# hidasib/GRU4Rec

Measured on AMD Instinct MI355X. Metric: mini-batches/sec (gru4rec.py:661), RSC15-shaped batch=128 n_sample=2048 BPR-max, higher is better.
Workload: dtype f32

## Files before the change

### gru4rec_amd/build.py

```python
import glob
import os
import subprocess
import sys

HERE = os.path.dirname(os.path.abspath(__file__))
SRC = os.path.join(HERE, 'csrc', 'g4r_api.hip')
SRC_HOST = os.path.join(HERE, 'csrc', 'g4r_io.cpp')
OUT = os.path.join(HERE, 'libgru4rec_hip.so')
DEPS = sorted(p for ext in ('hip', 'cuh', 'hpp', 'cpp') for p in glob.glob(os.path.join(HERE, 'csrc', '*.' + ext))) + \
       [os.path.join(os.path.dirname(HERE), 'include', 'gru4rec_hip.h'), os.path.abspath(__file__)]


def build(force=False, verbose=False, out=None, defs=(), flags=()):
    if out is not None:
        return _compile(out, list(defs), verbose, list(flags))
    if not force and os.path.exists(OUT) and all(os.path.getmtime(OUT) >= os.path.getmtime(d) for d in DEPS):
        return OUT
    return _compile(OUT, [], verbose)


COMMON_FLAGS = ['-mllvm', '-amdgpu-kernarg-preload-count=16']


MUTANTS = {1: 'sparse accumulator increments x 1.01', 2: 'sparse Adagrad steps x 1.01', 3: 'dense accumulator increments x 1.01',
# ... 7 lines not shown
           10: "k_replay_final (g4r_recommend_sessions) reads every row's final state from the buffer of the chunk's LONGEST history",
           11: "k_score_cand (g4r_score_candidates*): a work item past a row's first slice reads the items of the row's first slice",
           12: "the two-stage top-k (g4r_recommend_*_scan) ranks its candidates by the APPROXIMATE bf16 scores: the fp32 re-scoring is skipped",
           13: "cosine (g4r_similar_items): the candidate's inverse norm is read at the candidate POSITION instead of its item index",
           14: "k_rollout_feed (g4r_continue_sessions): the sorted insertion drops an item that sorts ABOVE every item already in the row's "
               "exclusion list, so it is never excluded and can be generated again",
           15: "k_beam_advance (g4r_beam_sessions) reads the hidden state of beam row i ITSELF instead of the row of its parent: a new beam "
               "carries on from the wrong state wherever the selection re-parents",
           16: "the owner walk of k_sparse_update_generic drops the first hit of every pass after the first (an item with more than 64 "
               "earlier occurrences in a step loses one of them per later pass)",
           17: "opt_rule's new second statistic (adadelta's update average, Adam's mean) x 1.01",
           18: "k_loss_rows' grp_fast takes a group of V columns whose last column is the first inactive in-batch one (column M) as wholly "
               "active: the unmasked copy of the element loops runs over it",
           19: "k_loss_rows' first pass starts its loop past the prefetched groups one STEP late: the columns of the first trip keep "
               "whatever the LDS held",
           20: "gumbel_noise (g4r_sample_sessions) ignores the decoding step (Philox counter word 2 = 0): every step of a draw gets the "
               "noise of step 0",
           21: "k_owner_window takes the sample-store row of every step of its window from the window's FIRST global step: the owner "
               "tables of the later steps are those of another list",
           22: "hidden_act_bwd decides the branch of leaky / elu / selu on the VALUE of the stored candidate (c >= 0), not on its sign bit: "
               "a pre-activation whose result rounds to -0.0 gets the positive branch's slope",
           23: "hidden_act_bwd: the negative-branch slope of leaky / elu / selu x 1.01",
           24: "k_mmr_rerank (g4r_diversify_*): from the second update on, a position's largest similarity to the picks is OVERWRITTEN by "
               "its similarity to the last pick instead of max-ed with it"}


def mutant_path(k):
    return os.path.join(HERE, '_variants', 'libgru4rec_hip_mut%d.so' % k)


def build_mutants(force=False, verbose=False):
    import fcntl
    from concurrent.futures import ThreadPoolExecutor
    os.makedirs(os.path.join(HERE, '_variants'), exist_ok=True)

    def stale():
        return [k for k in MUTANTS if force or not os.path.exists(mutant_path(k)) or
                any(os.path.getmtime(mutant_path(k)) < os.path.getmtime(d) for d in DEPS)]
    if not stale():
        return [mutant_path(k) for k in MUTANTS]
    with open(os.path.join(HERE, '_variants', '.lock'), 'w') as lock:
        fcntl.flock(lock, fcntl.LOCK_EX)
        todo = stale()
        if todo:
            _host_object(verbose)
            with ThreadPoolExecutor(min(len(todo), 2)) as ex:
                list(ex.map(lambda k: _device(mutant_path(k), ['G4R_MUTATE=%d' % k], verbose, audit=(k != 4)), todo))
# ... 108 lines not shown
```

### gru4rec_amd/csrc/g4r_host_create.hpp

```cpp

int g4r_device_count(void) {
    int n = 0;
    if (hipGetDeviceCount(&n) != hipSuccess) return 0;
    return n;
}
const char* g4r_last_error(void) { return g_err.c_str(); }
#ifndef G4R_HIPCC_VERSION
#define G4R_HIPCC_VERSION "unknown"
#endif
const char* g4r_version(void) { return "gru4rec_hip 0.4 (gfx950; hipcc " G4R_HIPCC_VERSION "; isa-audited)"; }
int g4r_sizeof_config(void) { return (int)sizeof(g4r_config); }

static int build_lean_args(g4r_model* m) {
    DevModel& d = m->dm;
    const StepKernels& k = m->kern;
    const int L = d.n_layers;
    std::vector<LeanV> av(L); std::vector<LeanH> ah(L); std::vector<LeanDa> aa(L); std::vector<LeanDy> ay(L);
    const bool constrained = d.embed_mode == G4R_EMBED_CONSTRAINED;
    bool any_layer = false;
    for (int l = 0; l < L; ++l) {
        if (k.fwd[l] != FWD_LEAN) continue;
        any_layer = true;
        LeanV& v = av[l]; memset(&v, 0, sizeof(v));
        v.Wx = d.dense_p + d.offWx[l]; v.Wrz = d.dense_p + d.offWrz[l]; v.Bh = d.dense_p + d.offBh[l];
// ... 52 lines not shown
        u.lr = d.lr; u.mom = d.mom; u.lmbd = d.lmbd;
        m->h_leanU = u;
        const std::vector<DenseTile> tiles = dense_tiles(d, 16, 64);
        m->ntiles16 = (int)tiles.size();
        const size_t nslot = cdiv((long long)G4R_OWN_SLOTS * d.R * 16 * sizeof(int), (long long)sizeof(DenseTile));
        if (dalloc(m, &m->d_tiles16, tiles.size() + nslot) || dalloc(m, &m->d_leanU, (size_t)1)) return -1;
        d.own_pos = m->sw.owner_scan_in_update ? nullptr : (int*)(m->d_tiles16 + tiles.size());
        m->h_leanU.own_on = d.own_pos ? 1 : 0;
        const bool pays = cdiv(d.R, LOSS_NW) > G4R_OWN_WINDOW_MINWG;
        m->own_window = d.own_pos && d.R <= G4R_OWN_WINDOW_MAXR && (m->sw.owner_window > 0 || (m->sw.owner_window < 0 && pays));
        HIPCHK(hipMemcpyAsync(m->d_tiles16, tiles.data(), tiles.size() * sizeof(DenseTile), hipMemcpyHostToDevice, m->stream));
        HIPCHK(hipStreamSynchronize(m->stream));
    }
    HIPCHK(hipStreamSynchronize(m->stream));
    return 0;
}

static KernelSwitches read_switches(const g4r_config& cfg) {
    KernelSwitches w;
    w.no_lean = getenv("G4R_NO_LEAN") != nullptr; w.no_mt = getenv("G4R_NO_MT") != nullptr; w.no_bmt = getenv("G4R_NO_BMT") != nullptr;
    w.no_merge = getenv("G4R_NO_MERGE") != nullptr; w.owner_scan_in_update = env_int("G4R_OWNER_SCAN", 0) != 0;
    w.owner_window = env_int("G4R_OWNER_WINDOW", -1);
    w.score_b_split = env_int("G4R_SCORE_B_SPLIT", 1) != 0;
    w.allow_lean_update = env_int("G4R_LEAN_UPDATE", 1) != 0; w.defer = env_int("G4R_DEFER", cfg.defer_updates) != 0;
    w.p2_geo = env_int("G4R_P2_GEO", -1); w.ba_geo = env_int("G4R_BA_GEO", -1);
    w.wide2 = env_int("G4R_WIDE2", -1); w.p1_ks = env_int("G4R_P1_KS", 128); w.bb_ks = env_int("G4R_BB_KS", 0);
    const char* skip = getenv("G4R_SKIP_KN");
    w.skip_kn = skip ? strtoull(skip, nullptr, 0) : 0ull;
    w.trace = getenv("G4R_TRACE") != nullptr;
    return w;
}

int g4r_create(const g4r_config* cfg, g4r_model** out) {
    if (!cfg || !out) return fail("null argument");
    if (cfg->n_layers < 1 || cfg->n_layers > G4R_MAX_LAYERS) return fail("n_layers out of range");
    if (cfg->batch_size < 1 || cfg->n_items < 1) return fail("batch_size / n_items must be positive");
    for (int l = 0; l < cfg->n_layers; ++l)
        if (cfg->layers[l] % 4 != 0 || cfg->layers[l] < 4 || cfg->layers[l] > 1024)
            return fail("layer sizes must be multiples of 4 in [4, 1024]");
    if (cfg->embed_mode == G4R_EMBED_SEPARATE && (cfg->embedding % 4 != 0 || cfg->embedding < 4 || cfg->embedding > 1024))
        return fail("embedding must be a multiple of 4 in [4, 1024]");
    if (cfg->embed_mode != G4R_EMBED_CONSTRAINED && cfg->embed_mode != G4R_EMBED_SEPARATE && cfg->embed_mode != G4R_EMBED_ONEHOT)
        return fail("unsupported embedding mode");
    if (cfg->embed_mode == G4R_EMBED_ONEHOT && 3 * cfg->layers[0] > 1024)
        return fail("one-hot input: 3 * layers[0] must be <= 1024 (row width of the Wx[0] table)");
    if (cfg->loss < 0 || cfg->loss > G4R_LOSS_XE_LOGIT) return fail("unsupported loss");
// ... 224 lines not shown
```

### gru4rec_amd/csrc/g4r_host_debug.hpp

```cpp
int g4r_get_debug(g4r_model* m, const char* name, float* host, int64_t count) {
    if (!m || !name || !host) return fail("null argument");
    HIPCHK(hipSetDevice(m->cfg.device));
    DevModel& d = m->dm;
    const StepKernels& k = m->kern;
    std::string s(name);
    const float* p = nullptr; int64_t n = 0;
    int l = 0;
    if (!s.empty() && isdigit((unsigned char)s.back())) { l = s.back() - '0'; s.pop_back(); }
    if (l >= d.n_layers) return fail("layer out of range");
    const int64_t bd = (int64_t)d.B * d.D[l];
    if (s == "scores") { p = d.Sc; n = (int64_t)d.B * d.ldSc; }
    else if (s == "dSx") { p = d.dSx + (size_t)((m->gstep - 1) & d.defer_mask) * (size_t)d.dSx_stride; n = (int64_t)d.B * d.Ein; }
    else if (s == "dSy") { p = d.dSy + (size_t)((m->gstep - 1) & d.defer_mask) * (size_t)d.dSy_stride; n = (int64_t)d.ldSc * d.Dtop; }
    else if (s == "dSBy") { p = d.dSBy + (size_t)((m->gstep - 1) & d.defer_mask) * (size_t)d.dSBy_stride; n = d.ldSc; }
    else if (s == "defer_stats") {
        if (count < 4) return fail("count");
        double rows = 0, bias = 0;
        if (m->defer_on) {
            std::vector<unsigned> st(2048);
            HIPCHK(hipStreamSynchronize(m->stream));
            HIPCHK(hipMemcpy(st.data(), d.dstat, st.size() * sizeof(unsigned), hipMemcpyDeviceToHost));
            for (size_t i = 0; i < st.size(); i += 2) { rows += st[i]; bias += st[i + 1]; }
        }
        host[0] = (float)rows; host[1] = (float)bias; host[2] = m->defer_on ? 1.f : 0.f; host[3] = (float)(d.defer_mask + 1);
// ... 55 lines not shown
        host[0] = (float)(k.p2_deep[0] + 2 * k.ba_deep[0]); return 0;
    }
    else if (s == "score_mt") { if (count < 1) return fail("count"); host[0] = k.score_fwd == SF_MT ? 272.f : 0.f; return 0; }
    else if (s == "score_bmt") { if (count < 1) return fail("count"); host[0] = (float)k.bmt_slabs; return 0; }
    else if (s == "lean") {
        if (count < 4) return fail("count");
        int mk = 0;
        for (int l = 0; l < d.n_layers; ++l) mk |= k.fwd[l] == FWD_LEAN ? 1 << l : 0;
        host[0] = (float)mk; host[1] = k.score_fwd == SF_LEAN ? 1.f : 0.f; host[2] = k.score_bwd == SB_LEAN ? 1.f : 0.f;
        host[3] = k.update == UP_LEAN ? 1.f : 0.f;
        return 0;
    }
    else if (s == "kernels") {
        const int ML = G4R_MAX_LAYERS;
        const int tail[] = {k.score_fwd, k.loss_spec, k.loss_long, k.loss_quads, k.score_bwd, k.kch, k.ksplit, k.bmt_slabs, k.update, k.chunks, k.wide_dense, k.finish_rows};
        if (count < 4 * ML + 12) return fail("count");
        for (int i = 0; i < 4 * ML + 12; ++i) host[i] = i < 4 * ML ? 0.f : (float)tail[i - 4 * ML];
        for (int l = 0; l < d.n_layers; ++l) {
            host[l] = (float)k.fwd[l]; host[ML + l] = (float)k.bwd[l]; host[2 * ML + l] = (float)(k.p2_deep[l] + 2 * k.ba_deep[l]); host[3 * ML + l] = (float)k.wg[l].use;
        }
        return 0;
    }
    else if (s == "generic") { if (count < 1) return fail("count"); host[0] = (float)d.generic; return 0; }
    else if (s == "score_b_split") { if (count < 1) return fail("count"); host[0] = (float)k.score_a_host; return 0; }
    else if (s == "n_cu") { if (count < 1) return fail("count"); host[0] = (float)m->n_cu; return 0; }
    else if (s == "ksplit") { if (count < 1) return fail("count"); host[0] = (float)d.ksplit; return 0; }
    else if (s == "dev_syncs") { if (count < 1) return fail("count"); host[0] = (float)m->n_dev_syncs; return 0; }
    else if (s == "dense_count") { if (count < 1) return fail("count"); host[0] = (float)d.dense_count; return 0; }
    else if (s == "occ_score_tile") {
        if (count < 1) return fail("count");
        int nb = 0;
        for (size_t lds = SMEM_SF2; lds >= SMEM_SF2 - 2048; lds -= 512) {
            HIPCHK(hipOccupancyMaxActiveBlocksPerMultiprocessor(&nb, (const void*)k_score_fwd_t2, GT_NTH, lds));
            fprintf(stderr, "[g4r] k_score_fwd_t2 dynamic LDS %zu -> %d workgroups per CU\n", lds, nb);
        }
        host[0] = (float)nb;
        return 0;
    }
    else if (s == "graph_mode") {
        if (count < 1) return fail("count");
        host[0] = m->gexec ? 1.f : (m->gexec_head ? 2.f : 0.f);
        return 0;
    }
    else return fail(std::string("unknown debug buffer ") + name);
    if (count != n) return fail(std::string("size mismatch for debug buffer ") + name + " expected " + std::to_string(n));
    HIPCHK(hipStreamSynchronize(m->stream));
// ... 169 lines not shown
```

### gru4rec_amd/csrc/g4r_host_model.hpp

```cpp
static thread_local std::string g_err;
static int fail(const std::string& s) { g_err = s; return -1; }
void g4r_set_error(const char* fmt, ...) {
    char buf[1024];
    va_list ap;
    va_start(ap, fmt);
    vsnprintf(buf, sizeof(buf), fmt, ap);
    va_end(ap);
    g_err = buf;
}
#define HIPCHK(x)                                                                                        \
    do {                                                                                                 \
        hipError_t e_ = (x);                                                                             \
        if (e_ != hipSuccess)                                                                            \
            return fail(std::string(#x) + ": " + hipGetErrorString(e_) + " @" + std::to_string(__LINE__)); \
    } while (0)
#define NCCLCHK(x)                                                                                         \
    do {                                                                                                   \
        ncclResult_t e_ = (x);                                                                             \
        if (e_ != ncclSuccess)                                                                             \
            return fail(std::string(#x) + ": " + ncclGetErrorString(e_) + " @" + std::to_string(__LINE__)); \
    } while (0)

enum { KN_GRU_P1 = 0, KN_GRU_P2, KN_SCORE_FWD, KN_LOSS, KN_SCORE_BWD, KN_BWD_PRE, KN_BWD_A, KN_BWD_B, KN_DENSE, KN_ALLREDUCE,
       KN_DENSE_APPLY, KN_SPARSE, KN_UPDATE, KN_BWD_FUSED, KN_FWD_FUSED, KN_GATE, KN_FLUSH, KN_SCAN, KN_FINISH, KN_GRU_V, KN_GRU_H, KN_GRU_DA, KN_GRU_DY, KN_OWNER_WINDOW, KN_COUNT };
static const char* KN_NAMES[KN_COUNT] = {"k_gru_p1", "k_gru_p2", "k_score_fwd", "k_loss_rows", "k_score_bwd", "k_gru_bwd_pre",
                                         "k_gru_bwd_a", "k_gru_bwd_b", "k_dense_grad", "rccl_allreduce", "k_dense_apply",
                                         "k_sparse_update", "k_update", "k_gru_bwd", "k_gru_fwd", "k_gru_gate", "k_sparse_flush", "k_defer_scan", "k_finish_rows", "k_gru_v", "k_gru_h", "k_gru_da", "k_gru_dy", "k_owner_window"};

struct EvRec { int kn; hipEvent_t a, b; };

struct KernelSwitches {
    bool no_lean = false;
    bool no_mt = false, no_bmt = false;
    bool no_merge = false;
    bool allow_lean_update = true;
    bool score_b_split = true;
    bool owner_scan_in_update = false;
    int owner_window = -1;
    bool defer = false;
    int p2_geo = -1, ba_geo = -1;
    int wide2 = -1, p1_ks = 128, bb_ks = 0;
    unsigned long long skip_kn = 0;
    bool trace = false;
};
enum GruFwdKind { FWD_LEAN = 0 , FWD_FUSED = 1 , FWD_P1S = 2 ,
                  FWD_P1_N64 = 3, FWD_P1_N32 = 4 };
enum GruBwdKind { BWD_LEAN = 0 , BWD_FUSED = 1 , BWD_ONEHOT = 2, BWD_BW = 3, BWD_B = 4 };
enum ScoreFwdKind { SF_LEAN = 0 , SF_MT = 1 , SF_T3 = 2, SF_T2 = 3, SF_K64 = 4, SF_K128 = 5  };
enum ScoreBwdKind { SB_LEAN = 0 , SB_BMT = 1 , SB_BWD2 = 2 , SB_W = 3, SB_N = 4  };
enum UpdateKind { UP_LEAN = 0 , UP_MERGED = 1 , UP_SPLIT = 2 };
struct WideGeo { int use = 0, ny = 1, nh = 1, kys = 0, khs = 0, bbn = 1, bbk = 0; };
struct StepKernels {
    int fwd[G4R_MAX_LAYERS], bwd[G4R_MAX_LAYERS];
    int p2_deep[G4R_MAX_LAYERS], ba_deep[G4R_MAX_LAYERS];
    WideGeo wg[G4R_MAX_LAYERS];
    int score_fwd;
    int loss_spec, loss_long, loss_quads;
    int score_bwd;
    int score_a_host;
    int kch, ksplit;
    int bmt_slabs;
    int nblkA, nblkB, ndtA, ndtB, nrtB;
    int update;
    int chunks;
    int wide_dense;
    int finish_rows;
};

template <class T>
struct DevBuf {
    T* p = nullptr;
    int64_t cap = 0;
    int reserve(g4r_model* m, int64_t n);
};

struct g4r_model {
    g4r_config cfg;
    DevModel dm;
    DevModel* d_dm = nullptr;
    int n_cu = 256;
    KernelSwitches sw;
    StepKernels kern;
// ... 323 lines not shown
    const bool wide = (B >= 256 && d.ldSc >= 4096) || (Dt % 64 == 0 && B >= 192 && d.ldSc >= 2048);
    const bool dma = Dt % 32 == 0 && (wide || (Dt >= 256 && B >= 64 && d.ldSc >= 1024));
    bool mt = false;
    if (!sw.no_mt && dma && Dt % 32 == 0 && Dt >= 32 && n_cu / cdiv(B, 64) >= 1) {
        const int nrb = cdiv(B, 64), W = 16 * cdiv(d.ldSc, 16 * (n_cu / nrb));
        mt = W == 272 && nrb * cdiv(d.ldSc, W) * 8 >= n_cu * 7;
    }
    const bool lean_s = !sw.no_lean && Dt <= LN_MAXD && Dt % 4 == 0 && !wide && !dma && B < 65536 && d.ldSc < 65536;
    k.score_fwd = lean_s ? SF_LEAN : mt ? SF_MT : dma ? SF_T3 : (wide && Dt % T2_BK == 0) ? SF_T2 : wide ? SF_K64 : SF_K128;
    k.loss_spec = (d.final_act == G4R_ACT_ELU && d.loss == G4R_LOSS_BPR_MAX) ? 1 : (d.final_act == G4R_ACT_SOFTMAX && d.loss == G4R_LOSS_XE) ? 2
                : (d.final_act == G4R_ACT_ELU && d.loss == G4R_LOSS_TOP1_MAX) ? 3 : 0;
    k.loss_long = (size_t)(2 * d.ldSc + 18 * LOSS_NW) * sizeof(float) > (size_t)(156 * 1024);
    k.loss_quads = d.ldSc >= 4 * LOSS_T;
    const bool bwd2 = wide && Dt % 64 == 0;
    const bool top_tiles = k.bwd[top] != BWD_LEAN && k.bwd[top] != BWD_FUSED;
    if (!sw.no_bmt && bwd2 && top_tiles && Dt % 128 == 0 && Dt <= 512 && d.ldSc % BMT_WA == 0 && d.ldSc <= 0xFFFF && B <= 0xFFFF) {
        const int ntA = d.ldSc / BMT_WA * (Dt / 32), den = cdiv(B, 64) * (Dt / 128), ks = ntA / den;
        if (ntA % den == 0 && ntA % 8 == 0 && ntA <= n_cu && ntA * 8 >= n_cu * 7 && BMT_WA % (Dt / 32) == 0 && 4 * (BMT_WA / (Dt / 32)) <= 256 &&
            ks >= 2 && ks <= 24 && d.ldSc % ks == 0 && (d.ldSc / ks) % 32 == 0 && d.ldSc / ks <= 2048)
            k.bmt_slabs = ks;
    }
    k.score_bwd = (lean_s && B <= 128) ? SB_LEAN : k.bmt_slabs ? SB_BMT : bwd2 ? SB_BWD2 : wide ? SB_W : SB_N;
    k.score_a_host = (sw.score_b_split && k.score_bwd == SB_LEAN && k.bwd[top] == BWD_LEAN) ? 1 : 0;
    const int slabs_target = top_tiles ? 17 : 9;
    k.kch = GT_BK * std::max(1, (cdiv(d.ldSc, GT_BK) + slabs_target / 2) / slabs_target);
    if (k.score_bwd == SB_LEAN) k.kch = 128;
    else if (k.score_bwd == SB_BMT) k.kch = d.ldSc / k.bmt_slabs;
    else if (k.score_bwd == SB_BWD2) {
        const int ndt = Dt / 64, nrt = cdiv(B, 64), nA = cdiv(d.ldSc, 64) * ndt;
        double best = 2.0;
        for (int ks = 12; ks <= 24; ++ks) {
            const int kch = (cdiv(d.ldSc, ks) + 7) & ~7;
            if (cdiv(d.ldSc, kch) != ks) continue;
            const double rounds = (double)(nA + ks * nrt * ndt) / n_cu;
            const double waste = (std::ceil(rounds) - rounds) / std::ceil(rounds) + 1e-3 * std::abs(ks - 17);
            if (waste < best) { best = waste; k.kch = kch; }
        }
    }
    k.ksplit = cdiv(d.ldSc, k.kch);
    const int TB = wide ? 64 : 32;
    k.ndtA = cdiv(Dt + 1, TB); k.nblkA = cdiv(d.ldSc, TB) * k.ndtA;
    k.ndtB = cdiv(Dt, TB); k.nrtB = cdiv(B, TB); k.nblkB = k.ksplit * k.nrtB * k.ndtB;
    const int w = std::max(Dt, d.Ein);
    k.chunks = w <= 256 ? 1 : (w <= 512 ? 2 : 4);
    const bool dy0_parts = (k.wg[0].use & 8) != 0;
    const bool merged = !d.generic && !sw.no_merge && k.chunks <= 2 && !k.wide_dense;
// ... 12 lines not shown
```

### gru4rec_amd/csrc/g4r_host_step.hpp

```cpp
extern "C++" {
struct StepLauncher {
    g4r_model* m;
    hipStream_t s;
    std::vector<EvRec>* recs;
    size_t evi = 0;
    int kn = -1;
    hipEvent_t ev_a = nullptr, ev_b = nullptr;
    StepLauncher(g4r_model* m_, std::vector<EvRec>* recs_) : m(m_), s(m_->stream), recs(recs_) {}
    void use(int kn_, hipEvent_t a, hipEvent_t b) { kn = kn_; ev_a = a; ev_b = b; }
    void open(int kn_) {
        if (m->sw.trace) { fprintf(stderr, "[g4r] launch %s\n", KN_NAMES[kn_]); fflush(stderr); }
        use(kn_, nullptr, nullptr);
        if (!recs) return;
        while (m->evs.size() < evi + 2) { hipEvent_t e; (void)hipEventCreate(&e); m->evs.push_back(e); }
        use(kn_, m->evs[evi], m->evs[evi + 1]);
        evi += 2;
        recs->push_back(EvRec{kn_, ev_a, ev_b});
    }
    bool skipped() const { return m->sw.skip_kn && kn >= 0 && ((m->sw.skip_kn >> kn) & 1ull); }
    template <class... P, class... A>
    void launch(void (*kern)(P...), dim3 grid, dim3 block, size_t smem, A... a) {
        if (skipped()) return;
        if (ev_a) hipExtLaunchKernelGGL(kern, grid, block, (unsigned)smem, s, ev_a, ev_b, 0, static_cast<P>(a)...);
        else hipLaunchKernelGGL(kern, grid, block, smem, s, static_cast<P>(a)...);
// ... 119 lines not shown
    default: lk.launch(k_score_bwd_n, dim3(k.nblkA + k.nblkB), dim3(GT_NTH), std::max(SMEM_TN, SMEM_NN) + (size_t)d.kch * sizeof(int), dmp, stp, k.nblkA, k.ndtA, k.ndtB, k.nrtB); break;
    }
    lk.close();
}

static void gru_backward(g4r_model* m, StepLauncher& lk, int l) {
    const DevModel& d = m->dm;
    const StepKernels& k = m->kern;
    const int L = d.n_layers, B = d.B;
    const DevModel* dmp = (const DevModel*)m->d_dm;
    StepState* stp = (StepState*)d.st;
    if (k.bwd[l] == BWD_LEAN) {
        const int nrb = cdiv(B, 16), gx = cdiv(d.IN[l], 16);
        const int* meta = d.cur_in + 2 * B;
        const LeanDa& q = m->h_leanDa[l];
        const LeanDy& y = m->h_leanDy[l];
        const unsigned dims = (unsigned)d.D[l] | ((unsigned)d.IN[l] << 16);
        lk.open(KN_GRU_DA);
        lk.launch(k_gru_da, dim3(cdiv(d.D[l], 16), nrb), dim3(128), 0, m->d_leanDa + l, meta, q.dsrc, q.Wh, q.z, q.c, q.H0, q.H1, (unsigned)d.D[l] | ((unsigned)q.ks << 16), B);
        lk.close();
        lk.open(KN_GRU_DY);
        if (score_a_hosted(m, lk) && l == L - 1) {
            const LeanB& b = m->h_leanB;
            lk.launch(k_gru_dy_a, dim3(gx, nrb + cdiv(cdiv(b.nA, 2), gx)), dim3(1024), 0, m->d_leanDy + l, meta, y.occ_idx, y.dV, y.drp, y.Wx, y.r, dims, B, m->d_leanB, d.cur_col,
                      d.Sc, d.hd[L - 1], d.accWy, (unsigned)d.Dtop | ((unsigned)B << 16), (unsigned)d.N | ((unsigned)d.ldSc << 16), (unsigned)b.nA | ((unsigned)b.ndh << 16));
        } else lk.launch(k_gru_dy, dim3(gx, nrb), dim3(1024), 0, m->d_leanDy + l, meta, y.occ_idx, y.dV, y.drp, y.Wx, y.r, dims, B);
        lk.close();
        return;
    }
    if (k.bwd[l] == BWD_FUSED) {
        lk.open(KN_BWD_FUSED);
        lk.launch(k_gru_bwd_fused, dim3(cdiv(d.IN[l], 32), cdiv(B, BF_ROWS)), dim3(512), smem_bwd_fused(d.D[l]), dmp, stp, l);
        lk.close();
        return;
    }
    lk.open(KN_BWD_PRE);
    lk.launch(k_gru_bwd_pre, dim3(cdiv((long long)B * d.D[l], 256)), dim3(256), 0, dmp, stp, l);
    lk.close();
    lk.open(KN_BWD_A);
    dim3 ga(cdiv(d.D[l], GT_BN), cdiv(B, GT_BM));
    int nfin = 0;
    if (l == L - 1 && k.score_bwd == SB_BMT) { nfin = cdiv(cdiv(d.N, 16), (int)ga.x); ga.y += nfin; }
    if (k.ba_deep[l]) lk.launch(k_gru_bwd_a_w8d, ga, dim3(512), SMEM_BA_256, dmp, stp, l, nfin);
    else lk.launch(k_gru_bwd_a_w4, ga, dim3(GT_NTH), SMEM_NT, dmp, stp, l, nfin);
    lk.close();
    lk.open(KN_BWD_B);
    const WideGeo& G = k.wg[l];
    if (k.bwd[l] == BWD_ONEHOT) lk.launch(k_onehot_step, dim3(cdiv((long long)B * d.Ein, 4 * 256)), dim3(256), 0, dmp, stp);
    else if (k.bwd[l] == BWD_BW) lk.launch(k_gru_bwd_bw, dim3(cdiv(d.IN[l], 64) * cdiv(B, 64) * G.bbn), dim3(256), SMEM_T3, dmp, stp, l, G.bbn, G.bbk);
// ... 437 lines not shown
```

### gru4rec_amd/csrc/g4r_lean_kernels.cuh

```cuda
#pragma once

#define LN_MAXD 128

__device__ __forceinline__ float ldu(const GAS float* base, unsigned boff) { return *(const GAS float*)((const GAS char*)base + boff); }
__device__ __forceinline__ int ldu_i(const GAS int* base, unsigned boff) { return *(const GAS int*)((const GAS char*)base + boff); }
__device__ __forceinline__ float4 ldu4(const GAS float* base, unsigned boff) { return *(const GAS float4*)((const GAS char*)base + boff); }
__device__ __forceinline__ void stu(GAS float* base, unsigned boff, float v) { *(GAS float*)((GAS char*)base + boff) = v; }
__device__ __forceinline__ void stu4(GAS float* base, unsigned boff, float4 v) { *(GAS float4*)((GAS char*)base + boff) = v; }

#if defined(G4R_CLK_TRACE)
#define LCLK_INIT(dbgp, slot) GAS long long* clk_ = ((dbgp) && blockIdx.x == 1 && blockIdx.y == 1 && blockIdx.z == 0 && threadIdx.x == 0) ? (dbgp) + (slot) : nullptr
#define LCLK(i) do { if (clk_) clk_[i] = wall_clock64(); } while (0)
#define LCLK_USE(x) do { if (clk_ && (x) == 123.456f) clk_[15] = 0; } while (0)
#define LSPAN_BEGIN(tilep, base) GAS long long* span_ = ((tilep) && threadIdx.x == 0) ? (tilep) + 8 * (size_t)((base) + (blockIdx.z * gridDim.y + blockIdx.y) * gridDim.x + blockIdx.x) : nullptr; \
    if (span_) span_[0] = wall_clock64()
#define LSPAN_END() do { if (span_) span_[1] = wall_clock64(); } while (0)
#define LSPAN_BEGIN_AT(tilep, idx, lead) GAS long long* span_ = ((tilep) && (lead)) ? (tilep) + 8 * (size_t)(idx) : nullptr; \
    if (span_) span_[0] = wall_clock64()
#else
#define LCLK_INIT(dbgp, slot)
#define LCLK(i)
#define LCLK_USE(x)
#define LSPAN_BEGIN(tilep, base)
#define LSPAN_END()
#define LSPAN_BEGIN_AT(tilep, idx, lead)
#endif

struct LeanV {
    GP(const float) Wx; GP(const float) Wrz; GP(const float) Bh; GP(const float) H0; GP(const float) H1;
    GP(const float) ysrc;
    GP(const int) cur_in;
// ... 335 lines not shown
    for (int q = 0; q < 4; ++q) acc[q] = (f32x4){0.f, 0.f, 0.f, 0.f};
#pragma unroll
    for (int q = 0; q < 4; ++q) acc[q] = mfma16(bq[q].x, da[0], acc[q]);
#pragma unroll
    for (int q = 0; q < 4; ++q) acc[q] = mfma16(bq[q].y, da[1], acc[q]);
#pragma unroll
    for (int q = 0; q < 4; ++q) acc[q] = mfma16(bq[q].z, da[2], acc[q]);
#pragma unroll
    for (int q = 0; q < 4; ++q) acc[q] = mfma16(bq[q].w, da[3], acc[q]);
    LCLK_USE(acc[0][0]); LCLK(5);
    if ((int)row < M) {
        const unsigned ob = j * ps + 4 * (row * D + 4 * lg);
#pragma unroll
        for (int q = 0; q < 4; ++q) {
            const unsigned n = 16 * (4 * wid + q) + 4 * lg;
            if (n < D) stu4(a.drp, ob + 64 * (4 * wid + q), make_float4(acc[q][0], acc[q][1], acc[q][2], acc[q][3]));
        }
    }
    LCLK(6);
    LSPAN_END();
}

#define LN_PL 8
__device__ __forceinline__ void gru_dy_tile(const LeanDy* __restrict__ ap, const int* meta_, const int* occ_idx_, const float* dV_, const float* drp_,
                                            const float* Wx_, const float* r_, const unsigned dims, const unsigned B, float* sJ) {
    const unsigned tid = threadIdx.x, lane = tid & 63, li = lane & 15, lg = lane >> 4;
    const unsigned wid = __builtin_amdgcn_readfirstlane(tid >> 6);
    const unsigned D = dims & 0xFFFFu, IN = dims >> 16, Dq = D >> 2;
    const unsigned m0 = blockIdx.y * 16, row = m0 + li, rowB = min(row, B - 1);
    const unsigned ncol = 16 * blockIdx.x + li, nc = min(ncol, IN - 1);
    const unsigned rowe = m0 + 4 * lg + (wid & 3);
    const GAS float* Wx = (const GAS float*)Wx_;
#if defined(G4R_CLK_TRACE)
    const long long tk0 = wall_clock64();
    GAS long long* ck = nullptr;
#define DYCK(i) do { if (ck) ck[i] = wall_clock64(); } while (0)
#else
#define DYCK(i)
#endif
    f32x4 acc;
    int4 mt;
    float a2 = 0.f;
    int cnt2 = 0, itm = -1;
    LeanState sx;
    if (wid < 8) {
        if (wid < 4) itm = ldu_i((const GAS int*)occ_idx_, 4 * min(rowe, B - 1));
        mt = ldi4((const GAS int*)meta_);
        const unsigned part = (wid >> 2) * 2;
        const unsigned Q0 = 8 * (wid & 3) + lg, Q1 = Q0 + 4;
        const bool ok0 = Q0 < Dq, ok1 = Q1 < Dq;
        const unsigned Qa = ok0 ? Q0 : 0, Qb = ok1 ? Q1 : 0;
        const unsigned offw = 4 * (nc * 3 * D + part * D), offa = 4 * (rowB * 3 * D + part * D);
        float4 a0 = ldu4((const GAS float*)dV_, offa + 16 * Qa), a1 = ldu4((const GAS float*)dV_, offa + 16 * Qb);
        const float4 b0 = ldu4(Wx, offw + 16 * Qa), b1 = ldu4(Wx, offw + 16 * Qb);
        const LeanDy a = *ap;
        lean_pin(a.accT, a.occ_fl, a.n_items, a.layer0);
#if defined(G4R_CLK_TRACE)
        ck = (a.dbg && blockIdx.x == 1 && blockIdx.y == 1 && tid == 0) ? a.dbg + 32 : nullptr;
        if (ck) ck[0] = tk0;
#endif
        DYCK(1);
        if (a.layer0 && wid < 4) {
            const unsigned ic = min((unsigned)max(itm, 0), (unsigned)a.n_items - 1);
            a2 = a.accT[(size_t)ic * IN + nc];
            cnt2 = a.occ_fl[4 * (size_t)ic + 2];
        }
        DYCK(2);
        sx = lean_state(mt);
        DYCK(3);
        const bool rowok = (int)row < sx.M;
        if (!(ok0 && rowok)) a0 = make_float4(0.f, 0.f, 0.f, 0.f);
        if (!(ok1 && rowok)) a1 = make_float4(0.f, 0.f, 0.f, 0.f);
        f32x4 acc0 = (f32x4){0.f, 0.f, 0.f, 0.f}, acc1 = (f32x4){0.f, 0.f, 0.f, 0.f};
        acc0 = mfma16(a0.x, b0.x, acc0);
        acc1 = mfma16(a0.y, b0.y, acc1);
        acc0 = mfma16(a0.z, b0.z, acc0);
        acc1 = mfma16(a0.w, b0.w, acc1);
        acc0 = mfma16(a1.x, b1.x, acc0);
        acc1 = mfma16(a1.y, b1.y, acc1);
        acc0 = mfma16(a1.z, b1.z, acc0);
        acc1 = mfma16(a1.w, b1.w, acc1);
        acc = acc0 + acc1;
#if defined(G4R_CLK_TRACE)
        if (ck) { if (acc[0] == 123.4f) ck[15] = 0; ck[4] = wall_clock64(); }
#endif
    } else {
        mt = ldi4((const GAS int*)meta_);
        const unsigned Q0 = 4 * (wid - 8) + lg;
        const bool ok0 = Q0 < Dq;
        const unsigned Qa = ok0 ? Q0 : 0;
        const unsigned offr = 4 * (rowB * D + 4 * Qa), NTD = (D + 15) >> 4, ps = 4 * B * D;
        float4 pv[LN_PL];
#pragma unroll
        for (int q = 0; q < LN_PL; ++q) pv[q] = ldu4((const GAS float*)drp_, offr + min((unsigned)q, NTD - 1) * ps);
        const float4 r4 = ldu4((const GAS float*)r_, offr);
        const float4 b0 = ldu4(Wx, 4 * (nc * 3 * D + D) + 16 * Qa);
        const LeanDy a = *ap;
        lean_pin(a.H0, a.H1, a.dV);
#if defined(G4R_CLK_TRACE)
        ck = (a.dbg && blockIdx.x == 1 && blockIdx.y == 1 && tid == 512) ? a.dbg + 40 : nullptr;
        if (ck) ck[0] = tk0;
#endif
        DYCK(1);
        const float4 h40 = ldu4(a.H0, offr), h41 = ldu4(a.H1, offr);
        float4 s = make_float4(0.f, 0.f, 0.f, 0.f);
#pragma unroll
        for (int q = 0; q < LN_PL; ++q) {
            const float w = ((unsigned)q < NTD) ? 1.f : 0.f;
            s.x = fmaf(w, pv[q].x, s.x); s.y = fmaf(w, pv[q].y, s.y); s.z = fmaf(w, pv[q].z, s.z); s.w = fmaf(w, pv[q].w, s.w);
        }
        DYCK(2);
        sx = lean_state(mt);
        const float4 h4 = (sx.g & 1u) ? h41 : h40;
        s.x *= h4.x * r4.x * (1.f - r4.x); s.y *= h4.y * r4.y * (1.f - r4.y);
        s.z *= h4.z * r4.z * (1.f - r4.z); s.w *= h4.w * r4.w * (1.f - r4.w);
        const bool rowok = (int)row < sx.M;
        if (blockIdx.x == 0 && ok0 && rowok) stu4(a.dV, 4 * (row * 3 * D + D + 4 * Qa), s);
        if (!(ok0 && rowok)) s = make_float4(0.f, 0.f, 0.f, 0.f);
        f32x4 acc0 = (f32x4){0.f, 0.f, 0.f, 0.f}, acc1 = (f32x4){0.f, 0.f, 0.f, 0.f};
        acc0 = mfma16(s.x, b0.x, acc0);
        acc1 = mfma16(s.y, b0.y, acc1);
        acc0 = mfma16(s.z, b0.z, acc0);
        acc1 = mfma16(s.w, b0.w, acc1);
        acc = acc0 + acc1;
#if defined(G4R_CLK_TRACE)
        if (ck) { if (acc[0] == 123.4f) ck[7] = 0; ck[3] = wall_clock64(); }
#endif
    }
    const int M = sx.M;
    if ((int)m0 >= M) return;
#pragma unroll
    for (int rg = 0; rg < 4; ++rg) sJ[(rg * 16 + wid) * 64 + lane] = acc[rg];
    __syncthreads();
    if (wid >= 4) return;
    const LeanDy a = *ap;
    LCLK_INIT(a.dbg, 48); LCLK(6);
    LSPAN_BEGIN(a.dbgtile, 1500);
#if defined(G4R_CLK_TRACE)
    if (span_) { span_[2] = span_[0]; span_[0] = tk0; }
#endif
    float v = 0.f;
#pragma unroll
    for (int w = 0; w < 16; ++w) v += sJ[(wid * 16 + w) * 64 + lane];
    if (ncol >= IN || (int)rowe >= M) return;
    const unsigned o = 4 * (rowe * IN + ncol);
    if (a.layer0) {
        if (a.drop_e > 0.f) v *= drop_mult(a.seed, sx.g, G4R_STREAM_DROP_EMBED, rowe, ncol, 1.0f - a.drop_e);
        const float an = a2 + G4R_MUT_ACC(v * v);
        GAS float* dSx = a.dSx + (size_t)(sx.g & (unsigned)a.defer_mask) * (size_t)a.dSx_stride;
        stu(dSx, o, a.generic ? v : G4R_MUT_STEP(a.lr * v * frsq(an + G4R_EPS_ADAGRAD)));
        if (!a.generic && cnt2 == 1 && itm >= 0) a.accT[(size_t)itm * IN + ncol] = an;
        else stu(a.dAx, o, an);
    } else {
        stu(a.dylo, o, v);
    }
    LCLK(7);
    LSPAN_END();
}
__global__ __launch_bounds__(1024) void k_gru_dy(const LeanDy* __restrict__ ap, const int* meta_, const int* occ_idx_, const float* dV_, const float* drp_,
                                                 const float* Wx_, const float* r_, unsigned dims, unsigned B) {
    __shared__ float sJ[4 * 16 * 64];
    gru_dy_tile(ap, meta_, occ_idx_, dV_, drp_, Wx_, r_, dims, B, sJ);
}

template <bool LOGQ>
__global__ __launch_bounds__(256) void k_score_s(const LeanS* __restrict__ ap, const int* meta_, const int* cur_col_, const float* hd_, const float* Wy_,
                                                 const float* By_, float* Sc_, unsigned dimsA, unsigned dimsB) {
    __shared__ f32x4 sJ[4 * 4 * 64];
    const unsigned tid = threadIdx.x, lane = tid & 63, li = lane & 15, lg = lane >> 4;
    const unsigned wid = __builtin_amdgcn_readfirstlane(tid >> 6);
    const unsigned D = dimsA & 0xFFFFu, B = dimsA >> 16, N = dimsB & 0xFFFFu, ldSc = dimsB >> 16, Dq = D >> 2;
    const unsigned n0 = blockIdx.x * 32, m0 = blockIdx.y * 32;
    const GAS int* cur_col = (const GAS int*)cur_col_;
    const unsigned nA = n0 + li, nB = n0 + 16 + li;
    int it0 = ldu_i(cur_col, 4 * min(nA, ldSc - 1)), it1 = ldu_i(cur_col, 4 * min(nB, ldSc - 1));
    const int4 mt = ldi4((const GAS int*)meta_);
    const unsigned Q0 = 8 * wid + lg, Q1 = Q0 + 4;
    const bool ok0 = Q0 < Dq, ok1 = Q1 < Dq;
    const unsigned Qa = ok0 ? Q0 : 0, Qb = ok1 ? Q1 : 0;
    const GAS float* hd = (const GAS float*)hd_;
    const unsigned ra = 4 * (min(m0 + li, B - 1) * D), rb = 4 * (min(m0 + 16 + li, B - 1) * D);
    float4 a00 = ldu4(hd, ra + 16 * Qa), a01 = ldu4(hd, ra + 16 * Qb), a10 = ldu4(hd, rb + 16 * Qa), a11 = ldu4(hd, rb + 16 * Qb);
    const LeanS a = *ap;
    lean_pin(a.col_item, a.occ_idx, a.occ_fl, a.R, a.pub_fl, a.logq, a.dbg);
    LCLK_INIT(a.dbg, 56); LCLK(0);
    LSPAN_BEGIN(a.dbgtile, 4096);
// ... 194 lines not shown
}

template <bool ROLE_A>
__global__ __launch_bounds__(512) void k_score_b(const LeanB* __restrict__ ap, const int* meta_, const int* cur_col_, const float* Sc_, const float* hd_,
                                                 const float* Wy_, float* accWy_, unsigned dimsA, unsigned dimsB) {
    __shared__ f32x4 sJ[4 * 8 * 64];
    const unsigned tid = threadIdx.x, lane = tid & 63;
    const unsigned wid = __builtin_amdgcn_readfirstlane(tid >> 6);
    const unsigned D = dimsA & 0xFFFFu, B = dimsA >> 16, N = dimsB & 0xFFFFu, ldSc = dimsB >> 16;
    const GAS int* cur_col = (const GAS int*)cur_col_;
    const GAS float *Sc = (const GAS float*)Sc_, *hd = (const GAS float*)hd_;
    const int4 mt = ldi4((const GAS int*)meta_);
    const LeanB a = *ap;
    if (ROLE_A) {
        if (blockIdx.x < (unsigned)a.nA) { score_b_role_a(a, mt, cur_col, Sc, hd, accWy_, D, B, N, ldSc, blockIdx.x, (unsigned)a.ndh, wid, lane, sJ, true, tid == 0); return; }
        score_b_role_b(a, mt, cur_col, Sc, Wy_, D, B, ldSc, blockIdx.x - (unsigned)a.nA, wid, lane, sJ);
    } else {
        score_b_role_b(a, mt, cur_col, Sc, Wy_, D, B, ldSc, blockIdx.x, wid, lane, sJ);
    }
}
template __global__ void k_score_b<true>(const LeanB*, const int*, const int*, const float*, const float*, const float*, float*, unsigned, unsigned);
template __global__ void k_score_b<false>(const LeanB*, const int*, const int*, const float*, const float*, const float*, float*, unsigned, unsigned);

__global__ __launch_bounds__(1024) void k_gru_dy_a(const LeanDy* __restrict__ ap, const int* meta_, const int* occ_idx_, const float* dV_, const float* drp_,
                                                   const float* Wx_, const float* r_, unsigned dims, unsigned B, const LeanB* __restrict__ bp,
                                                   const int* cur_col_, const float* Sc_, const float* hd_, float* accWy_, unsigned dimsA, unsigned dimsB, unsigned tilesA) {
    __shared__ f32x4 sJ[2 * 4 * 8 * 64];
    const unsigned nrb = (B + 15) >> 4;
    if (blockIdx.y < nrb) { gru_dy_tile(ap, meta_, occ_idx_, dV_, drp_, Wx_, r_, dims, B, (float*)sJ); return; }
    const unsigned tid = threadIdx.x, lane = tid & 63;
    const unsigned wid = __builtin_amdgcn_readfirstlane(tid >> 6);
    const unsigned nA = tilesA & 0xFFFFu, half = wid >> 3;
    const unsigned t0 = 2 * ((blockIdx.y - nrb) * gridDim.x + blockIdx.x), t = t0 + half;
    if (t0 >= nA) return;
    const int4 mt = ldi4((const GAS int*)meta_);
    const LeanB a = *bp;
    const bool live = t < nA;
    score_b_role_a(a, mt, (const GAS int*)cur_col_, (const GAS float*)Sc_, (const GAS float*)hd_, accWy_, dimsA & 0xFFFFu, dimsA >> 16, dimsB & 0xFFFFu,
                   dimsB >> 16, live ? t : nA - 1, tilesA >> 16, wid & 7, lane, sJ + half * (4 * 8 * 64), live, (tid & 511) == 0);
}

template <bool MOM>
__device__ __forceinline__ void lean_rows_update(const LeanU& a, const GAS int* occ_idx, GAS int* occ_fl, const GAS float* dSx, const GAS float* dSy,
                                                 const GAS float* dSBy, const GAS int* opos_t, unsigned k, unsigned R, unsigned B) {
    const unsigned lane = threadIdx.x & 63;
    const bool tableE = k < B && !a.constrained;
    const unsigned W = tableE ? (unsigned)a.wE : (unsigned)a.wY, nc4 = W >> 2;
    const unsigned c4 = min(lane, nc4 - 1);
    const bool lok = lane < nc4;
    const unsigned kc = min(k, R - 1);
    int item = ldu_i(occ_idx, 4 * kc);
    const int opos = ldu_i(opos_t, 4 * (16 * kc + min(lane, 15u)));
    const GAS float* srow = (kc < B) ? dSx + (size_t)kc * W : dSy + (size_t)(kc - B) * W;
    const float4 sk = ld4(srow + 4 * c4);
    const bool bias = k >= B;
    const float bsk = bias ? dSBy[kc - B] : 0.f;
    lean_pin(a.Wy, a.E, a.accWy, a.accE, a.By, a.accBy, a.dAx, a.dAy, a.dABy, a.n_items, a.lr, a.mom, a.lmbd);
    if (k >= R) item = -1;
    GAS float* P = tableE ? a.E : a.Wy;
    GAS float* A = tableE ? a.accE : a.accWy;
    GAS float* V = tableE ? a.velE : a.velWy;
    const unsigned ic = (unsigned)max(item, 0);
    GAS int* flp = occ_fl + 4 * ((tableE ? (size_t)a.n_items : 0) + ic);
// ... 267 lines not shown
```

Baseline: 26860.

## Stage GRU dy dr' operand through LDS with coalesced buffer loads

In the dy kernel, waves 8-15 now load the partial dr' planes, r and the hidden state with coalesced row-major buffer loads, one float4 per thread. They reduce the planes and apply the reset-gate derivative, then stage the result in LDS. After a barrier each wave reads its fragment back for the MFMA, replacing the previous per-fragment strided global loads. The combined dy/score kernel also puts the score-A blocks first in the grid and the dy tiles last, which changes scheduling order. The cost is an extra barrier and more LDS in the plain kernel, and the reversed-order mutant is added for testing.

```diff
diff --git a/gru4rec_amd/build.py b/gru4rec_amd/build.py
--- a/gru4rec_amd/build.py
+++ b/gru4rec_amd/build.py
@@ -53,7 +53,9 @@
                "a pre-activation whose result rounds to -0.0 gets the positive branch's slope",
            23: "hidden_act_bwd: the negative-branch slope of leaky / elu / selu x 1.01",
            24: "k_mmr_rerank (g4r_diversify_*): from the second update on, a position's largest similarity to the picks is OVERWRITTEN by "
-               "its similarity to the last pick instead of max-ed with it"}
+               "its similarity to the last pick instead of max-ed with it",
+           25: "k_gru_dy's staged dr' operand (gru_dy_tile<true>) adds the partial planes of k_gru_da in REVERSE order: the sum's last bits "
+               "differ from the fragment-layout form's (G4R_DY_STAGE=0)"}
 
 
 def mutant_path(k):
diff --git a/gru4rec_amd/csrc/g4r_host_create.hpp b/gru4rec_amd/csrc/g4r_host_create.hpp
--- a/gru4rec_amd/csrc/g4r_host_create.hpp
+++ b/gru4rec_amd/csrc/g4r_host_create.hpp
@@ -98,6 +98,7 @@
     w.no_merge = getenv("G4R_NO_MERGE") != nullptr; w.owner_scan_in_update = env_int("G4R_OWNER_SCAN", 0) != 0;
     w.owner_window = env_int("G4R_OWNER_WINDOW", -1);
     w.score_b_split = env_int("G4R_SCORE_B_SPLIT", 1) != 0;
+    w.dy_stage = env_int("G4R_DY_STAGE", 1) != 0;
     w.allow_lean_update = env_int("G4R_LEAN_UPDATE", 1) != 0; w.defer = env_int("G4R_DEFER", cfg.defer_updates) != 0;
     w.p2_geo = env_int("G4R_P2_GEO", -1); w.ba_geo = env_int("G4R_BA_GEO", -1);
     w.wide2 = env_int("G4R_WIDE2", -1); w.p1_ks = env_int("G4R_P1_KS", 128); w.bb_ks = env_int("G4R_BB_KS", 0);
diff --git a/gru4rec_amd/csrc/g4r_host_debug.hpp b/gru4rec_amd/csrc/g4r_host_debug.hpp
--- a/gru4rec_amd/csrc/g4r_host_debug.hpp
+++ b/gru4rec_amd/csrc/g4r_host_debug.hpp
@@ -101,6 +101,7 @@
         return 0;
     }
     else if (s == "generic") { if (count < 1) return fail("count"); host[0] = (float)d.generic; return 0; }
+    else if (s == "dy_stage") { if (count < 1) return fail("count"); host[0] = (float)k.dy_stage; return 0; }
     else if (s == "score_b_split") { if (count < 1) return fail("count"); host[0] = (float)k.score_a_host; return 0; }
     else if (s == "n_cu") { if (count < 1) return fail("count"); host[0] = (float)m->n_cu; return 0; }
     else if (s == "ksplit") { if (count < 1) return fail("count"); host[0] = (float)d.ksplit; return 0; }
diff --git a/gru4rec_amd/csrc/g4r_host_model.hpp b/gru4rec_amd/csrc/g4r_host_model.hpp
--- a/gru4rec_amd/csrc/g4r_host_model.hpp
+++ b/gru4rec_amd/csrc/g4r_host_model.hpp
@@ -35,6 +35,7 @@
     bool no_merge = false;
     bool allow_lean_update = true;
     bool score_b_split = true;
+    bool dy_stage = true;
     bool owner_scan_in_update = false;
     int owner_window = -1;
     bool defer = false;
@@ -58,6 +59,7 @@
     int loss_spec, loss_long, loss_quads;
     int score_bwd;
     int score_a_host;
+    int dy_stage;
     int kch, ksplit;
     int bmt_slabs;
     int nblkA, nblkB, ndtA, ndtB, nrtB;
@@ -427,6 +429,7 @@
     }
     k.score_bwd = (lean_s && B <= 128) ? SB_LEAN : k.bmt_slabs ? SB_BMT : bwd2 ? SB_BWD2 : wide ? SB_W : SB_N;
     k.score_a_host = (sw.score_b_split && k.score_bwd == SB_LEAN && k.bwd[top] == BWD_LEAN) ? 1 : 0;
+    k.dy_stage = sw.dy_stage ? 1 : 0;
     const int slabs_target = top_tiles ? 17 : 9;
     k.kch = GT_BK * std::max(1, (cdiv(d.ldSc, GT_BK) + slabs_target / 2) / slabs_target);
     if (k.score_bwd == SB_LEAN) k.kch = 128;
diff --git a/gru4rec_amd/csrc/g4r_host_step.hpp b/gru4rec_amd/csrc/g4r_host_step.hpp
--- a/gru4rec_amd/csrc/g4r_host_step.hpp
+++ b/gru4rec_amd/csrc/g4r_host_step.hpp
@@ -165,9 +165,9 @@
         lk.open(KN_GRU_DY);
         if (score_a_hosted(m, lk) && l == L - 1) {
             const LeanB& b = m->h_leanB;
-            lk.launch(k_gru_dy_a, dim3(gx, nrb + cdiv(cdiv(b.nA, 2), gx)), dim3(1024), 0, m->d_leanDy + l, meta, y.occ_idx, y.dV, y.drp, y.Wx, y.r, dims, B, m->d_leanB, d.cur_col,
+            lk.launch(k.dy_stage ? k_gru_dy_a<true> : k_gru_dy_a<false>, dim3(gx, nrb + cdiv(cdiv(b.nA, 2), gx)), dim3(1024), 0, m->d_leanDy + l, meta, y.occ_idx, y.dV, y.drp, y.Wx, y.r, dims, B, m->d_leanB, d.cur_col,
                       d.Sc, d.hd[L - 1], d.accWy, (unsigned)d.Dtop | ((unsigned)B << 16), (unsigned)d.N | ((unsigned)d.ldSc << 16), (unsigned)b.nA | ((unsigned)b.ndh << 16));
-        } else lk.launch(k_gru_dy, dim3(gx, nrb), dim3(1024), 0, m->d_leanDy + l, meta, y.occ_idx, y.dV, y.drp, y.Wx, y.r, dims, B);
+        } else lk.launch(k.dy_stage ? k_gru_dy<true> : k_gru_dy<false>, dim3(gx, nrb), dim3(1024), 0, m->d_leanDy + l, meta, y.occ_idx, y.dV, y.drp, y.Wx, y.r, dims, B);
         lk.close();
         return;
     }
diff --git a/gru4rec_amd/csrc/g4r_lean_kernels.cuh b/gru4rec_amd/csrc/g4r_lean_kernels.cuh
--- a/gru4rec_amd/csrc/g4r_lean_kernels.cuh
+++ b/gru4rec_amd/csrc/g4r_lean_kernels.cuh
@@ -7,6 +7,19 @@
 __device__ __forceinline__ float4 ldu4(const GAS float* base, unsigned boff) { return *(const GAS float4*)((const GAS char*)base + boff); }
 __device__ __forceinline__ void stu(GAS float* base, unsigned boff, float v) { *(GAS float*)((GAS char*)base + boff) = v; }
 __device__ __forceinline__ void stu4(GAS float* base, unsigned boff, float4 v) { *(GAS float4*)((GAS char*)base + boff) = v; }
+#define LN_OOB 0x80000000u
+#if defined(__HIP_DEVICE_COMPILE__)
+typedef __amdgpu_buffer_rsrc_t LeanRsrc;
+__device__ __forceinline__ LeanRsrc lean_rsrc(const void* base, unsigned bytes) { return __builtin_amdgcn_make_buffer_rsrc((void*)base, (short)0, (int)bytes, 0x00020000); }
+__device__ __forceinline__ float4 ldr4(LeanRsrc rs, unsigned boff) {
+    const f32x4 v = __builtin_bit_cast(f32x4, __builtin_amdgcn_raw_buffer_load_b128(rs, (int)boff, 0, 0));
+    return make_float4(v[0], v[1], v[2], v[3]);
+}
+#else
+typedef const void* LeanRsrc;
+__device__ __forceinline__ LeanRsrc lean_rsrc(const void* base, unsigned) { return base; }
+__device__ __forceinline__ float4 ldr4(LeanRsrc, unsigned) { return make_float4(0.f, 0.f, 0.f, 0.f); }
+#endif
 
 #if defined(G4R_CLK_TRACE)
 #define LCLK_INIT(dbgp, slot) GAS long long* clk_ = ((dbgp) && blockIdx.x == 1 && blockIdx.y == 1 && blockIdx.z == 0 && threadIdx.x == 0) ? (dbgp) + (slot) : nullptr
@@ -388,12 +401,15 @@
 }
 
 #define LN_PL 8
+#define LN_DYJ (4 * 16 * 64)
+template <bool STAGE>
 __device__ __forceinline__ void gru_dy_tile(const LeanDy* __restrict__ ap, const int* meta_, const int* occ_idx_, const float* dV_, const float* drp_,
-                                            const float* Wx_, const float* r_, const unsigned dims, const unsigned B, float* sJ) {
+                                            const float* Wx_, const float* r_, const unsigned dims, const unsigned B, const unsigned y0, float* sJ) {
     const unsigned tid = threadIdx.x, lane = tid & 63, li = lane & 15, lg = lane >> 4;
     const unsigned wid = __builtin_amdgcn_readfirstlane(tid >> 6);
     const unsigned D = dims & 0xFFFFu, IN = dims >> 16, Dq = D >> 2;
-    const unsigned m0 = blockIdx.y * 16, row = m0 + li, rowB = min(row, B - 1);
+    const unsigned by = blockIdx.y - y0;
+    const unsigned m0 = by * 16, row = m0 + li, rowB = min(row, B - 1);
     const unsigned ncol = 16 * blockIdx.x + li, nc = min(ncol, IN - 1);
     const unsigned rowe = m0 + 4 * lg + (wid & 3);
     const GAS float* Wx = (const GAS float*)Wx_;
@@ -408,6 +424,8 @@
     int4 mt;
     float a2 = 0.f;
     int cnt2 = 0, itm = -1;
+    float4 bS = make_float4(0.f, 0.f, 0.f, 0.f);
+    GAS float* dVs = nullptr;
     LeanState sx;
     if (wid < 8) {
         if (wid < 4) itm = ldu_i((const GAS int*)occ_idx_, 4 * min(rowe, B - 1));
@@ -422,7 +440,7 @@
         const LeanDy a = *ap;
         lean_pin(a.accT, a.occ_fl, a.n_items, a.layer0);
 #if defined(G4R_CLK_TRACE)
-        ck = (a.dbg && blockIdx.x == 1 && blockIdx.y == 1 && tid == 0) ? a.dbg + 32 : nullptr;
+        ck = (a.dbg && blockIdx.x == 1 && by == 1 && tid == 0) ? a.dbg + 32 : nullptr;
         if (ck) ck[0] = tk0;
 #endif
         DYCK(1);
@@ -450,6 +468,44 @@
 #if defined(G4R_CLK_TRACE)
         if (ck) { if (acc[0] == 123.4f) ck[15] = 0; ck[4] = wall_clock64(); }
 #endif
+    } else if (STAGE) {
+        mt = ldi4((const GAS int*)meta_);
+        const unsigned i4 = tid - 512, NTD = (D + 15) >> 4, ps = 4 * B * D;
+        const unsigned n4 = (min(m0 + 16, B) - m0) * Dq;
+        const unsigned offs = (i4 < n4) ? 4 * m0 * D + 16 * i4 : LN_OOB;
+        const LeanRsrc rp = lean_rsrc(drp_, NTD * ps), rr = lean_rsrc(r_, ps);
+        float4 pv[LN_PL];
+#pragma unroll
+        for (int q = 0; q < LN_PL; ++q) pv[q] = ldr4(rp, ((unsigned)q < NTD) ? offs + (unsigned)q * ps : LN_OOB);
+        const float4 r4 = ldr4(rr, offs);
+        const unsigned Qa = min(4 * (wid - 8) + lg, Dq - 1);
+        bS = ldu4(Wx, 4 * (nc * 3 * D + D) + 16 * Qa);
+        const LeanDy a = *ap;
+        lean_pin(a.H0, a.H1, a.dV);
+        dVs = a.dV;
+#if defined(G4R_CLK_TRACE)
+        ck = (a.dbg && blockIdx.x == 1 && by == 1 && tid == 512) ? a.dbg + 40 : nullptr;
+        if (ck) ck[0] = tk0;
+#endif
+        DYCK(1);
+        const float4 h40 = ldr4(lean_rsrc((const float*)a.H0, ps), offs), h41 = ldr4(lean_rsrc((const float*)a.H1, ps), offs);
+        float4 s = make_float4(0.f, 0.f, 0.f, 0.f);
+#if defined(G4R_MUTATE) && G4R_MUTATE == 25
+#pragma unroll
+        for (int q = LN_PL - 1; q >= 0; --q) {
+#else
+#pragma unroll
+        for (int q = 0; q < LN_PL; ++q) {
+#endif
+            const float w = ((unsigned)q < NTD) ? 1.f : 0.f;
+            s.x = fmaf(w, pv[q].x, s.x); s.y = fmaf(w, pv[q].y, s.y); s.z = fmaf(w, pv[q].z, s.z); s.w = fmaf(w, pv[q].w, s.w);
+        }
+        sx = lean_state(mt);
+        const float4 h4 = (sx.g & 1u) ? h41 : h40;
+        s.x *= h4.x * r4.x * (1.f - r4.x); s.y *= h4.y * r4.y * (1.f - r4.y);
+        s.z *= h4.z * r4.z * (1.f - r4.z); s.w *= h4.w * r4.w * (1.f - r4.w);
+        ((float4*)(sJ + LN_DYJ))[i4] = s;
+        DYCK(2);
     } else {
         mt = ldi4((const GAS int*)meta_);
         const unsigned Q0 = 4 * (wid - 8) + lg;
@@ -464,7 +520,7 @@
         const LeanDy a = *ap;
         lean_pin(a.H0, a.H1, a.dV);
 #if defined(G4R_CLK_TRACE)
-        ck = (a.dbg && blockIdx.x == 1 && blockIdx.y == 1 && tid == 512) ? a.dbg + 40 : nullptr;
+        ck = (a.dbg && blockIdx.x == 1 && by == 1 && tid == 512) ? a.dbg + 40 : nullptr;
         if (ck) ck[0] = tk0;
 #endif
         DYCK(1);
@@ -495,13 +551,41 @@
     }
     const int M = sx.M;
     if ((int)m0 >= M) return;
+    if (STAGE) {
+        __syncthreads();
+        if (wid >= 8) {
+            DYCK(3);
+            const unsigned Q0 = 4 * (wid - 8) + lg;
+            const bool ok0 = Q0 < Dq;
+            const unsigned Qa = ok0 ? Q0 : 0;
+            float4 s = ((const float4*)(sJ + LN_DYJ))[li * Dq + Qa];
+#if defined(G4R_CLK_TRACE)
+            if (ck) { if (s.x == 123.4f) ck[7] = 0; ck[4] = wall_clock64(); }
+#endif
+            const bool rowok = (int)row < M;
+            if (blockIdx.x == 0 && ok0 && rowok) stu4(dVs, 4 * (row * 3 * D + D + 4 * Qa), s);
+            if (!(ok0 && rowok)) s = make_float4(0.f, 0.f, 0.f, 0.f);
+            f32x4 acc0 = (f32x4){0.f, 0.f, 0.f, 0.f}, acc1 = (f32x4){0.f, 0.f, 0.f, 0.f};
+            acc0 = mfma16(s.x, bS.x, acc0);
+            acc1 = mfma16(s.y, bS.y, acc1);
+            acc0 = mfma16(s.z, bS.z, acc0);
+            acc1 = mfma16(s.w, bS.w, acc1);
+            acc = acc0 + acc1;
+#if defined(G4R_CLK_TRACE)
+            if (ck) { if (acc[0] == 123.4f) ck[7] = 0; ck[5] = wall_clock64(); }
+#endif
+        }
+    }
 #pragma unroll
     for (int rg = 0; rg < 4; ++rg) sJ[(rg * 16 + wid) * 64 + lane] = acc[rg];
     __syncthreads();
     if (wid >= 4) return;
     const LeanDy a = *ap;
-    LCLK_INIT(a.dbg, 48); LCLK(6);
-    LSPAN_BEGIN(a.dbgtile, 1500);
+#if defined(G4R_CLK_TRACE)
+    GAS long long* clk_ = (a.dbg && blockIdx.x == 1 && by == 1 && threadIdx.x == 0) ? a.dbg + 48 : nullptr;
+#endif
+    LCLK(6);
+    LSPAN_BEGIN_AT(a.dbgtile, 1500 + by * gridDim.x + blockIdx.x, threadIdx.x == 0);
 #if defined(G4R_CLK_TRACE)
     if (span_) { span_[2] = span_[0]; span_[0] = tk0; }
 #endif
@@ -523,11 +607,14 @@
     LCLK(7);
     LSPAN_END();
 }
+template <bool STAGE>
 __global__ __launch_bounds__(1024) void k_gru_dy(const LeanDy* __restrict__ ap, const int* meta_, const int* occ_idx_, const float* dV_, const float* drp_,
                                                  const float* Wx_, const float* r_, unsigned dims, unsigned B) {
-    __shared__ float sJ[4 * 16 * 64];
-    gru_dy_tile(ap, meta_, occ_idx_, dV_, drp_, Wx_, r_, dims, B, sJ);
-}
+    __shared__ float sJ[LN_DYJ + (STAGE ? 4 * 512 : 0)];
+    gru_dy_tile<STAGE>(ap, meta_, occ_idx_, dV_, drp_, Wx_, r_, dims, B, 0u, sJ);
+}
+template __global__ void k_gru_dy<false>(const LeanDy*, const int*, const int*, const float*, const float*, const float*, const float*, unsigned, unsigned);
+template __global__ void k_gru_dy<true>(const LeanDy*, const int*, const int*, const float*, const float*, const float*, const float*, unsigned, unsigned);
 
 template <bool LOGQ>
 __global__ __launch_bounds__(256) void k_score_s(const LeanS* __restrict__ ap, const int* meta_, const int* cur_col_, const float* hd_, const float* Wy_,
@@ -768,16 +855,18 @@
 template __global__ void k_score_b<true>(const LeanB*, const int*, const int*, const float*, const float*, const float*, float*, unsigned, unsigned);
 template __global__ void k_score_b<false>(const LeanB*, const int*, const int*, const float*, const float*, const float*, float*, unsigned, unsigned);
 
+template <bool STAGE>
 __global__ __launch_bounds__(1024) void k_gru_dy_a(const LeanDy* __restrict__ ap, const int* meta_, const int* occ_idx_, const float* dV_, const float* drp_,
                                                    const float* Wx_, const float* r_, unsigned dims, unsigned B, const LeanB* __restrict__ bp,
                                                    const int* cur_col_, const float* Sc_, const float* hd_, float* accWy_, unsigned dimsA, unsigned dimsB, unsigned tilesA) {
     __shared__ f32x4 sJ[2 * 4 * 8 * 64];
     const unsigned nrb = (B + 15) >> 4;
-    if (blockIdx.y < nrb) { gru_dy_tile(ap, meta_, occ_idx_, dV_, drp_, Wx_, r_, dims, B, (float*)sJ); return; }
+    const unsigned nra = gridDim.y - nrb;
+    if (blockIdx.y >= nra) { gru_dy_tile<STAGE>(ap, meta_, occ_idx_, dV_, drp_, Wx_, r_, dims, B, nra, (float*)sJ); return; }
     const unsigned tid = threadIdx.x, lane = tid & 63;
     const unsigned wid = __builtin_amdgcn_readfirstlane(tid >> 6);
     const unsigned nA = tilesA & 0xFFFFu, half = wid >> 3;
-    const unsigned t0 = 2 * ((blockIdx.y - nrb) * gridDim.x + blockIdx.x), t = t0 + half;
+    const unsigned t0 = 2 * (blockIdx.y * gridDim.x + blockIdx.x), t = t0 + half;
     if (t0 >= nA) return;
     const int4 mt = ldi4((const GAS int*)meta_);
     const LeanB a = *bp;
@@ -785,6 +874,10 @@
     score_b_role_a(a, mt, (const GAS int*)cur_col_, (const GAS float*)Sc_, (const GAS float*)hd_, accWy_, dimsA & 0xFFFFu, dimsA >> 16, dimsB & 0xFFFFu,
                    dimsB >> 16, live ? t : nA - 1, tilesA >> 16, wid & 7, lane, sJ + half * (4 * 8 * 64), live, (tid & 511) == 0);
 }
+template __global__ void k_gru_dy_a<false>(const LeanDy*, const int*, const int*, const float*, const float*, const float*, const float*, unsigned, unsigned, const LeanB*,
+                                           const int*, const float*, const float*, float*, unsigned, unsigned, unsigned);
+template __global__ void k_gru_dy_a<true>(const LeanDy*, const int*, const int*, const float*, const float*, const float*, const float*, unsigned, unsigned, const LeanB*,
+                                          const int*, const float*, const float*, float*, unsigned, unsigned, unsigned);
 
 template <bool MOM>
 __device__ __forceinline__ void lean_rows_update(const LeanU& a, const GAS int* occ_idx, GAS int* occ_fl, const GAS float* dSx, const GAS float* dSy,
```

Measured after the change: 26850. No clear change (-0.0%).
